# MCG-NJU/MotionRAG

Measured on AMD Instinct MI355X. Metric: denoise_step_frames_per_sec, higher is better.
Workload: dtype bf16

## Files before the change

### motionrag_amd/csrc/gemm_common.h

```cpp
#pragma once
#include <type_traits>
#include "common.h"
#include "../../include/mrag_hip.h"

namespace {

struct GemmP {
  const bf16_t* A; const bf16_t* W; const bf16_t* bias; bf16_t* C; const bf16_t* resid;
  const bf16_t* gate0; const bf16_t* gate1;
  long long M, N, K, lda, ldw, ldc, ldr, rows_per_batch, split, gate_stride;
  int tiles_m, tiles_n, group_m, staged, tuning;
  const bf16_t* qg; const bf16_t* qb; const bf16_t* kg; const bf16_t* kb; const float* rcos; const float* rsin;
  long long qk_D; int rope_text_len, qk_first; float qk_eps, q_premul;
  int cv_H, cv_W, cv_Hi, cv_Wi, cv_Ho, cv_Wo, cv_stride, cv_up, cv_ctiles, cv_T, cv_pad;
  long long cv_C, cv_HW;
  float acc_scale;
  float* sk_part; unsigned* sk_ticket;
  int sk_main, sk_rem, sk_units, sk_maxparts;
  const bf16_t* lna_g; const bf16_t* lna_b; float lna_eps; int lna;
  int tile_limit;
  int wb_tiles_m;
  long long w_bstride;
  int cv_lds;
  int cv_tf;
  long long cv_fs;
};

constexpr int SK_CUS = 256, SK_TICKET_BYTES = 1024;
constexpr int SK_FLAG_OFF = 8 * 128 * 144;
constexpr int SKM_ROWS = 32;

__device__ __forceinline__ float sum8_dpp(float x) {
  x += __int_as_float(__builtin_amdgcn_update_dpp(0, __float_as_int(x), 0xB1, 0xF, 0xF, true));
  x += __int_as_float(__builtin_amdgcn_update_dpp(0, __float_as_int(x), 0x4E, 0xF, 0xF, true));
  x += __int_as_float(__builtin_amdgcn_update_dpp(0, __float_as_int(x), 0x141, 0xF, 0xF, true));
  return x;
}

__device__ __forceinline__ u32x4 qk_row_math(u32x4 val, const bool has_gamma, const bool has_beta, const float (&gam)[8], const float (&bet)[8], const float eps,
                                             const bool has_rope, const bool vid, const f32x4 (&t4)[4], const bool premul_on, const float premul) {
  float v[8];
#pragma unroll
  for (int e = 0; e < 4; ++e) { v[2 * e] = __uint_as_float(val[e] << 16); v[2 * e + 1] = __uint_as_float(val[e] & 0xffff0000u); }
  if (has_gamma) {
    float sum = 0.f;
#pragma unroll
    for (int e = 0; e < 8; ++e) sum += v[e];
    sum = sum8_dpp(sum);
    const float mean = sum * (1.0f / 64.0f);
    float sq = 0.f;
#pragma unroll
    for (int e = 0; e < 8; ++e) { v[e] -= mean; sq += v[e] * v[e]; }
    sq = sum8_dpp(sq);
    const float rstd = rsqrtf(sq * (1.0f / 64.0f) + eps);
#pragma unroll
    for (int e = 0; e < 8; ++e) v[e] = v[e] * rstd * gam[e];
    if (has_beta) {
#pragma unroll
      for (int e = 0; e < 8; ++e) v[e] += bet[e];
    }
  }
  if (has_rope) {
    const float cc[8] = {t4[0][0], t4[0][1], t4[0][2], t4[0][3], t4[1][0], t4[1][1], t4[1][2], t4[1][3]};
    const float ss[8] = {t4[2][0], t4[2][1], t4[2][2], t4[2][3], t4[3][0], t4[3][1], t4[3][2], t4[3][3]};
#pragma unroll
    for (int i2 = 0; i2 < 4; ++i2) {
      const float a = v[2 * i2], b2 = v[2 * i2 + 1];
      const float oa = a * cc[2 * i2] - b2 * ss[2 * i2];
      const float ob = b2 * cc[2 * i2 + 1] + a * ss[2 * i2 + 1];
      v[2 * i2] = vid ? oa : a;
      v[2 * i2 + 1] = vid ? ob : b2;
    }
  }
  if (premul_on) {
#pragma unroll
    for (int e = 0; e < 8; ++e) v[e] *= premul;
  }
#pragma unroll
  for (int e = 0; e < 4; ++e) val[e] = pack_bf2(v[2 * e], v[2 * e + 1]);
  return val;
}

constexpr int EPI_GEGLU_TANH = 8;
template <int EPI>
constexpr bool is_geglu = (EPI == MRAG_EPI_GEGLU || EPI == EPI_GEGLU_TANH);

template <int EPI>
__device__ __forceinline__ float epi_act(float v) {
  if constexpr (EPI == MRAG_EPI_GELU_TANH) return gelu_tanh_f(v);
  else if constexpr (EPI == MRAG_EPI_GELU_ERF) return gelu_erf_f(v);
  else if constexpr (EPI == MRAG_EPI_SILU) return silu_f(v);
  else return v;
}


inline bool rows_16B_aligned(const void* C, long long ldc, const void* resid, long long ldr) {
  return ldc % 8 == 0 && ((uintptr_t)C & 15) == 0 && (!resid || (ldr % 8 == 0 && ((uintptr_t)resid & 15) == 0));
}

inline int group_m_of(int tuning) { return ((tuning >> 8) & 0xff) ? ((tuning >> 8) & 0xff) : 4; }

template <class P>
inline int launch_dyn_lds(void (*kernel)(P), dim3 grid, dim3 block, size_t lds_bytes, hipStream_t stream, const P& params) {
  const hipError_t e = hipFuncSetAttribute((const void*)kernel, hipFuncAttributeMaxDynamicSharedMemorySize, (int)lds_bytes);
  if (e != hipSuccess) return (int)e;
  MRAG_LAUNCH(kernel, grid, block, lds_bytes, stream, params);
  return (int)hipGetLastError();
}

inline bool wide_n_pays(long long N, int tuning = 0) {
  if (tuning & MRAG_GEMM_TUNE_NO_WIDE) return false;
  const long long w256 = (N + 255) / 256 * 256, w320 = (N + 319) / 320 * 320;
  return w320 * 100 < w256 * 90;
}

inline long long round_cost(long long M, long long N, int BN) {
  const long long tiles = ((M + 255) / 256) * ((N + BN - 1) / BN);
  return ((tiles + 255) / 256) * BN;
}
inline bool wide_rounds_pay(long long M, long long N, int tuning = 0, bool tail_rect = false) {
  if (tuning & MRAG_GEMM_TUNE_NO_WIDE) return false;
  long long c256 = round_cost(M, N, 256);
  if (tail_rect) c256 = (((M + 255) / 256) * ((N + 255) / 256) / 256) * 256 + 128;
  return round_cost(M, N, 320) * 100 < c256 * 85;
}
inline bool short_rows_pay(long long M, long long N, int tuning = 0) {
  if (tuning & MRAG_GEMM_TUNE_NO_WIDE) return false;
  const long long t192 = ((M + 191) / 192) * ((N + 255) / 256), t256 = ((M + 255) / 256) * ((N + 255) / 256);
  const long long c192 = ((t192 + 255) / 256) * 192 * 108, c256 = ((t256 + 255) / 256) * 256 * 100;
  return c192 * 100 < c256 * 90 && round_cost(M, N, 320) * 100 >= round_cost(M, N, 256) * 85;
}

inline bool narrow_n_pays(long long N) {
  const long long r = N % 256;
  return r != 0 && r <= 128;
}

struct SkPlan {
  bool use = false;
  int n_main = 0, rem = 0, units = 0, maxparts = 0;
  size_t bytes = 0;
};
inline SkPlan plan_streamk(long long M, long long N, long long K) {
  SkPlan pl;
  const long long tiles = ((M + 255) / 256) * ((N + 255) / 256);
  const int nk = (int)(K / 64);
  if (tiles < SK_CUS || tiles > (1 << 24) || nk < 16 || nk > 4096) return pl;
  const int rem = (int)(tiles % SK_CUS);
  if (rem == 0 || rem > 208) return pl;
  pl.rem = rem; pl.n_main = (int)(tiles - rem);
  pl.units = rem * 4 < SK_CUS ? rem * 4 : SK_CUS;
  const long long I = (long long)rem * nk;
  for (int t = 0, u = 0; t < rem; ++t) {
    while ((long long)(u + 1) * I / pl.units <= (long long)t * nk) ++u;
    int v = u;
    while ((long long)(v + 1) * I / pl.units < (long long)(t + 1) * nk) ++v;
    pl.maxparts = pl.maxparts > v - u + 1 ? pl.maxparts : v - u + 1;
  }
  pl.bytes = SK_TICKET_BYTES + (size_t)rem * pl.maxparts * 256 * 256 * sizeof(float);
  pl.use = true;
  return pl;
}

constexpr int W4_TAIL_MAX = 32;
inline bool tail_rect_wanted(long long tiles, int epi, int tuning) {
  const int rem = (int)(tiles % SK_CUS);
  return (tuning & MRAG_GEMM_TUNE_TAIL_RECT) && tiles >= 2 * SK_CUS && rem != 0 && rem <= W4_TAIL_MAX &&
         (epi == MRAG_EPI_NONE || epi == MRAG_EPI_GELU_TANH || epi == MRAG_EPI_RESID);
}

enum { TILE_256x256_W16, TILE_128x128, TILE_256x320, TILE_256x256 };

}

#define MRAG_GEMM_LAUNCHER extern "C" __attribute__((visibility("hidden"))) int
MRAG_GEMM_LAUNCHER launch_tiled(hipStream_t s, const GemmP& p, int epi, int tile, const SkPlan* sk);
MRAG_GEMM_LAUNCHER launch_w4(hipStream_t s, const GemmP& p, int epi);
MRAG_GEMM_LAUNCHER launch_k320(hipStream_t s, const GemmP& p, int epi);
MRAG_GEMM_LAUNCHER launch_skinny(hipStream_t s, const GemmP& p, int epi);
```

### motionrag_amd/csrc/gemm_w4.hip

```cpp
#include "gemm_common.h"

namespace {

template <int EPI>
__device__ __forceinline__ void epilogue_w4(const GemmP& p, char* smem, f32x4 (&acc)[8][8], const long long bm0, const long long bn0, const int wave, const int wrow0,
                                            const int wcol0, const int lane_in, const long long Mend) {
  constexpr bool HAS_R = (EPI == MRAG_EPI_GATE_RESID || EPI == MRAG_EPI_RESID), HAS_G = (EPI == MRAG_EPI_GATE_RESID), QK = (EPI == MRAG_EPI_QKNORM_ROPE);
  int lane_e = lane_in;
  asm volatile("" : "+v"(lane_e));
  const int lane = lane_e;
  const int frag_row = lane & 15, frag_q = lane >> 4;
  const long long n0 = bn0 + wcol0 + frag_q * 4;
  const long long m0 = bm0 + wrow0;
  long long g_b = 0, g_pos = 0;
  if constexpr (HAS_G || QK) {
    g_b = m0 / p.rows_per_batch;
    g_pos = m0 - g_b * p.rows_per_batch;
  }
  if (m0 >= Mend || bn0 + wcol0 >= p.N) return;
  const int mrows = (int)(Mend - m0 < 128 ? Mend - m0 : 128);
  bool fast = p.staged && bn0 + wcol0 + 128 <= p.N;
  if constexpr (HAS_G) fast = fast && g_pos + mrows - 1 < p.rows_per_batch && ((g_pos < p.split) == (g_pos + mrows - 1 < p.split));
  auto add_resid = [&](u32x2 out, const u32x2 r2) __attribute__((always_inline)) -> u32x2 {
    out[0] = pack_bf2(__uint_as_float(out[0] << 16) + __uint_as_float(r2[0] << 16), __uint_as_float(out[0] & 0xffff0000u) + __uint_as_float(r2[0] & 0xffff0000u));
    out[1] = pack_bf2(__uint_as_float(out[1] << 16) + __uint_as_float(r2[1] << 16), __uint_as_float(out[1] & 0xffff0000u) + __uint_as_float(r2[1] & 0xffff0000u));
    return out;
  };
  auto acc_math = [&](const int i, const int j, const u32x2 b2, const u32x2 g2) __attribute__((always_inline)) -> u32x2 {
    float v[4] = {acc[i][j][0], acc[i][j][1], acc[i][j][2], acc[i][j][3]};
    v[0] += __uint_as_float(b2[0] << 16); v[1] += __uint_as_float(b2[0] & 0xffff0000u);
    v[2] += __uint_as_float(b2[1] << 16); v[3] += __uint_as_float(b2[1] & 0xffff0000u);
    if constexpr (EPI == MRAG_EPI_GELU_TANH) {
      const f32x2 lo = gelu_tanh_f2(f32x2{v[0], v[1]}), hi = gelu_tanh_f2(f32x2{v[2], v[3]});
      v[0] = lo[0]; v[1] = lo[1]; v[2] = hi[0]; v[3] = hi[1];
    } else {
#pragma unroll
      for (int e = 0; e < 4; ++e) v[e] = epi_act<EPI>(v[e]);
    }
    if constexpr (HAS_G) {
      v[0] *= __uint_as_float(g2[0] << 16); v[1] *= __uint_as_float(g2[0] & 0xffff0000u);
      v[2] *= __uint_as_float(g2[1] << 16); v[3] *= __uint_as_float(g2[1] & 0xffff0000u);
    }
    if constexpr (EPI == MRAG_EPI_RESID) {
#pragma unroll
      for (int e = 0; e < 4; ++e) v[e] *= p.acc_scale;
    }
    return u32x2{pack_bf2(v[0], v[1]), pack_bf2(v[2], v[3])};
  };
  if (fast) {
    u32x2 bias[8], gate[8];
#pragma unroll
    for (int j = 0; j < 8; ++j) {
      bias[j] = p.bias ? *(const u32x2*)(p.bias + n0 + 16 * j) : u32x2{0u, 0u};
      if constexpr (HAS_G) gate[j] = *(const u32x2*)((g_pos < p.split ? p.gate0 : p.gate1) + g_b * p.gate_stride + n0 + 16 * j);
      else gate[j] = u32x2{0u, 0u};
    }
    const int r4 = lane >> 4, chunk = lane & 15;
    const bf16_t* rbase = HAS_R ? p.resid + m0 * p.ldr + n0 : nullptr;
    bf16_t* cbase = p.C + (m0 + r4) * p.ldc + (bn0 + wcol0 + chunk * 8);
    char* wput = smem + 131072 + wave * 8192 + frag_row * 256 + (frag_q & 1) * 8;
    const char* wget = smem + 131072 + wave * 8192 + r4 * 256;
    const int xput = frag_q >> 1;
    int qk_which = 2;
    bool has_rope = false;
    const bf16_t *gm = nullptr, *bt = nullptr;
    float gam[8], bet[8];
    f32x4 qk_tab[QK ? 3 : 1][4];
    unsigned qk_video = 0;
    auto qk_fetch = [&](const int st) __attribute__((always_inline)) {
      if constexpr (QK) {
        const int row = 4 * st + r4;
        long long pos = g_pos + (row < mrows ? row : mrows - 1);
        while (pos >= p.rows_per_batch) pos -= p.rows_per_batch;
        const int rp = (int)pos - p.rope_text_len;
        if (rp >= 0) qk_video |= 1u << st;
        const long long ro = (long long)(rp > 0 ? rp : 0) * 64 + (chunk & 7) * 8;
        f32x4(&dst)[4] = qk_tab[st % 3];
        dst[0] = *(const f32x4*)(p.rcos + ro); dst[1] = *(const f32x4*)(p.rcos + ro + 4);
        dst[2] = *(const f32x4*)(p.rsin + ro); dst[3] = *(const f32x4*)(p.rsin + ro + 4);
      }
    };
    if constexpr (QK) {
      qk_which = p.qk_first + (int)((bn0 + wcol0) / p.qk_D);
      has_rope = p.rcos != nullptr && qk_which < 2;
#pragma unroll
      for (int e = 0; e < 8; ++e) { gam[e] = 1.f; bet[e] = 0.f; }
      if (qk_which < 2) {
        gm = qk_which ? p.kg : p.qg;
        bt = qk_which ? p.kb : p.qb;
        const int d0 = (chunk & 7) * 8;
        if (gm) {
          const u32x4 graw = *(const u32x4*)(gm + d0);
#pragma unroll
          for (int e = 0; e < 4; ++e) { gam[2 * e] = __uint_as_float(graw[e] << 16); gam[2 * e + 1] = __uint_as_float(graw[e] & 0xffff0000u); }
          if (bt) {
            const u32x4 braw = *(const u32x4*)(bt + d0);
#pragma unroll
            for (int e = 0; e < 4; ++e) { bet[2 * e] = __uint_as_float(braw[e] << 16); bet[2 * e + 1] = __uint_as_float(braw[e] & 0xffff0000u); }
          }
        }
      }
      if (has_rope) { qk_fetch(0); qk_fetch(1); qk_fetch(2); }
    }
    constexpr int RD = 2;
    u32x2 rr[RD][8];
    auto fetch = [&](const int i, const int slot) __attribute__((always_inline)) {
      if constexpr (HAS_R) {
        const int row = 16 * i + frag_row;
        const bf16_t* rrow = rbase + (long long)(row < mrows ? row : mrows - 1) * p.ldr;
#pragma unroll
        for (int j = 0; j < 8; ++j) rr[slot][j] = *(const u32x2*)(rrow + 16 * j);
      }
    };
    auto put = [&](const int i) __attribute__((always_inline)) {
#pragma unroll
      for (int j = 0; j < 8; ++j) {
        u32x2 out = acc_math(i, j, bias[j], gate[j]);
        if constexpr (HAS_R) out = add_resid(out, rr[i % RD][j]);
        *(u32x2*)(wput + (i & 1) * 4096 + (((2 * j + xput) ^ frag_row) * 16)) = out;
      }
    };
    auto get_store = [&](const int i) __attribute__((always_inline)) {
      u32x4 val[4];
#pragma unroll
      for (int q = 0; q < 4; ++q) val[q] = *(const u32x4*)(wget + (i & 1) * 4096 + q * 1024 + ((chunk ^ (q * 4 + r4)) * 16));
#pragma unroll
      for (int q = 0; q < 4; ++q) {
        if constexpr (QK) {
          const int st = 4 * i + q;
          if (qk_which < 2) {
            val[q] = qk_row_math(val[q], gm != nullptr, bt != nullptr, gam, bet, p.qk_eps, has_rope, (qk_video >> st) & 1u, qk_tab[st % 3], qk_which == 0 && p.q_premul != 1.0f, p.q_premul);
            if (has_rope && st + 3 < 32) qk_fetch(st + 3);
          }
        }
        if (16 * i + 4 * q + r4 < mrows) *(u32x4*)(cbase + (long long)(16 * i + 4 * q) * p.ldc) = val[q];
      }
    };
#pragma unroll
    for (int i = 0; i < RD - 1; ++i) fetch(i, i);
#pragma unroll
    for (int i = 0; i < 8; ++i) {
      __builtin_amdgcn_sched_barrier(0);
      if (i + RD - 1 < 8) fetch(i + RD - 1, (i + RD - 1) % RD);
      put(i);
      if (i > 0) get_store(i - 1);
    }
    __builtin_amdgcn_sched_barrier(0);
    get_store(7);
    return;
  }
  if constexpr (QK) return;
  auto ncol = [&](const int j) __attribute__((always_inline)) { const long long n = n0 + 16 * j; return n < p.N ? n : p.N - 4; };
#pragma unroll
  for (int i = 0; i < 8; ++i) {
    __builtin_amdgcn_sched_barrier(0);
    const long long m = m0 + i * 16 + frag_row;
    const bool mok = m < Mend;
    const long long mc = mok ? m : Mend - 1;
    const bf16_t* gate = nullptr;
    if constexpr (HAS_G) {
      long long b = g_b, pos = g_pos + (mc - m0);
      while (pos >= p.rows_per_batch) { pos -= p.rows_per_batch; ++b; }
      gate = (pos < p.split ? p.gate0 : p.gate1) + b * p.gate_stride;
    }
#pragma unroll
    for (int j = 0; j < 8; ++j) {
      const long long n = ncol(j);
      const u32x2 b2 = p.bias ? *(const u32x2*)(p.bias + n) : u32x2{0u, 0u};
      u32x2 g2 = u32x2{0u, 0u};
      if constexpr (HAS_G) g2 = *(const u32x2*)(gate + n);
      u32x2 out = acc_math(i, j, b2, g2);
      if constexpr (HAS_R) out = add_resid(out, *(const u32x2*)(p.resid + mc * p.ldr + n));
      if (mok && n0 + 16 * j < p.N) *(u32x2*)(p.C + mc * p.ldc + n) = out;
    }
  }
  __builtin_amdgcn_s_waitcnt(0x0070);
}

template <int EPI>
__device__ __forceinline__ void epilogue_w4_geglu(const GemmP& p, char* smem, f32x4 (&acc)[8][8], const long long bm0, const long long bn0, const int wave, const int wrow0,
                                                  const int wcol0, const int lane_in) {
  int lane_e = lane_in;
  asm volatile("" : "+v"(lane_e));
  const int lane = lane_e;
  const int frag_row = lane & 15, frag_q = lane >> 4;
  const long long m0 = bm0 + wrow0;
  if (m0 >= p.M || bn0 + wcol0 >= p.N) return;
  const int mrows = (int)(p.M - m0 < 128 ? p.M - m0 : 128);
  const long long n0 = bn0 + wcol0 + frag_q * 4;
  u32x2 bv[4], bg[4];
#pragma unroll
  for (int jj = 0; jj < 4; ++jj) {
    bv[jj] = p.bias ? *(const u32x2*)(p.bias + n0 + 32 * jj) : u32x2{0u, 0u};
    bg[jj] = p.bias ? *(const u32x2*)(p.bias + n0 + 32 * jj + 16) : u32x2{0u, 0u};
  }
  const int r8 = lane >> 3, chunk = lane & 7;
  bf16_t* cbase = p.C + (m0 + r8) * p.ldc + ((bn0 + wcol0) >> 1) + chunk * 8;
  char* wput = smem + 131072 + wave * 8192 + frag_row * 128 + (frag_q & 1) * 8;
  const char* wget = smem + 131072 + wave * 8192 + r8 * 128 + ((chunk ^ r8) * 16);
  const int xput = frag_q >> 1, sw = frag_row & 7;
  auto put = [&](const int i) __attribute__((always_inline)) {
#pragma unroll
    for (int jj = 0; jj < 4; ++jj) {
      float v[4] = {acc[i][2 * jj][0], acc[i][2 * jj][1], acc[i][2 * jj][2], acc[i][2 * jj][3]};
      float g[4] = {acc[i][2 * jj + 1][0], acc[i][2 * jj + 1][1], acc[i][2 * jj + 1][2], acc[i][2 * jj + 1][3]};
      v[0] += __uint_as_float(bv[jj][0] << 16); v[1] += __uint_as_float(bv[jj][0] & 0xffff0000u);
      v[2] += __uint_as_float(bv[jj][1] << 16); v[3] += __uint_as_float(bv[jj][1] & 0xffff0000u);
      g[0] += __uint_as_float(bg[jj][0] << 16); g[1] += __uint_as_float(bg[jj][0] & 0xffff0000u);
      g[2] += __uint_as_float(bg[jj][1] << 16); g[3] += __uint_as_float(bg[jj][1] & 0xffff0000u);
      geglu4<EPI == EPI_GEGLU_TANH>(v, g);
      *(u32x2*)(wput + (i & 1) * 2048 + (((2 * jj + xput) ^ sw) * 16)) = u32x2{pack_bf2(v[0], v[1]), pack_bf2(v[2], v[3])};
    }
  };
  auto get_store = [&](const int i) __attribute__((always_inline)) {
    u32x4 val[2];
#pragma unroll
    for (int q = 0; q < 2; ++q) val[q] = *(const u32x4*)(wget + (i & 1) * 2048 + q * 1024);
#pragma unroll
    for (int q = 0; q < 2; ++q)
      if (16 * i + 8 * q + r8 < mrows) *(u32x4*)(cbase + (long long)(16 * i + 8 * q) * p.ldc) = val[q];
  };
#pragma unroll
  for (int i = 0; i < 8; ++i) {
    __builtin_amdgcn_sched_barrier(0);
    put(i);
    if (i > 0) get_store(i - 1);
  }
  __builtin_amdgcn_sched_barrier(0);
  get_store(7);
}

template <int N, class F>
__device__ __forceinline__ void static_for(F&& f) {
  if constexpr (N > 0) {
    static_for<N - 1>(f);
    f(std::integral_constant<int, N - 1>{});
  }
}

__device__ __forceinline__ void tile_coords(const GemmP& p, const int L, int& tile_m, int& tile_n) {
  const int gw = p.group_m * p.tiles_n;
  const int first_m = (L / gw) * p.group_m;
  const int gsz = min(p.tiles_m - first_m, p.group_m);
  tile_m = first_m + (L % gw) % gsz;
  tile_n = (L % gw) / gsz;
}

template <int EPI, bool WB = false>
__global__ __launch_bounds__(256) void gemm_w4_kernel(const GemmP p) {
  extern __shared__ __attribute__((aligned(16))) char smem[];
  constexpr unsigned STAGE = 65536, WOFF = 32768;
  const int lane = threadIdx.x & 63, wave = threadIdx.x >> 6, wm = wave >> 1, wn = wave & 1;
  const int wave_s = __builtin_amdgcn_readfirstlane(wave);
  const int tiles = p.tile_limit, nk = (int)(p.K / 64), G = (int)gridDim.x;
  auto tile_origin = [&](const int tm, long long& bm0, long long& m_end, long long& w_off) __attribute__((always_inline)) {
    if constexpr (WB) {
      const int b = tm / p.wb_tiles_m;
      bm0 = (long long)b * p.rows_per_batch + (long long)(tm - b * p.wb_tiles_m) * 256;
      m_end = (long long)(b + 1) * p.rows_per_batch;
      w_off = (long long)b * p.w_bstride;
    } else {
      bm0 = (long long)tm * 256; m_end = p.M; w_off = 0;
    }
  };
  const int slot = xcd_remap((int)blockIdx.x, G);
  unsigned voff[16];
  const bf16_t *baseA = p.A, *baseW = p.W;
  int d_r = 0, d_kt = 0;
  bool d_valid = false;
  auto cursor_set = [&](const int r) __attribute__((always_inline)) {
    const int L = r * G + slot;
    d_valid = L < tiles;
    if (!d_valid) return;
    int tm, tn;
    tile_coords(p, L, tm, tn);
    long long bm0, m_end, w_off;
    tile_origin(tm, bm0, m_end, w_off);
    const long long bn0 = (long long)tn * 256;
    int lane_c = lane;
    asm volatile("" : "+v"(lane_c));
    const int prow = lane_c >> 3, pchk = (lane_c & 7) ^ prow;
#pragma unroll
    for (int i = 0; i < 16; ++i) {
      const int q = wave_s + 4 * i;
      long long r8 = (i < 8) ? 8 * q + prow : 8 * (q - 32) + prow;
      const long long lim = (i < 8) ? m_end - bm0 : p.N - bn0;
      r8 = r8 < lim ? r8 : lim - 1;
      voff[i] = (unsigned)((r8 * ((i < 8) ? p.lda : p.ldw) + pchk * 8) * 2);
    }
    baseA = p.A + bm0 * p.lda;
    baseW = p.W + w_off + bn0 * p.ldw;
  };
  auto advance = [&]() __attribute__((always_inline)) {
    if (!d_valid) return;
    if (d_kt + 1 < nk) { ++d_kt; return; }
    cursor_set(d_r + 1);
    if (d_valid) { ++d_r; d_kt = 0; }
  };
  const unsigned smem_u = (unsigned)(size_t)smem;
  const unsigned fr = lane & 15, fq = lane >> 4, swz = lane & 7;
  const unsigned c0 = ((fq + 0) ^ swz) * 16, c1 = ((fq + 4) ^ swz) * 16;
  const unsigned rowA = smem_u + (wm * 128 + fr) * 128, rowW = smem_u + WOFF + (wn * 128 + fr) * 128;
  f32x4 acc[8][8];
  u32x4 a0[8], w0[8], a1[8], w1[8];
#define MRAG_W4_MF(I, J, W, A) asm volatile("v_mfma_f32_16x16x32_bf16 %0, %1, %2, %0" : "+a"(acc[I][J]) : "v"(W[J]), "v"(A[I]))
#define MRAG_W4_RD(D, ADDR, OFF) asm volatile("ds_read_b128 %0, %1 offset:%2" : "=v"(D) : "v"(ADDR), "n"(OFF) : "memory")
#define MRAG_W4_LGKM0(W, A)                                                                                          \
      asm volatile("s_waitcnt lgkmcnt(0)"                                                                             \
                   : "+v"(W[0]), "+v"(W[1]), "+v"(W[2]), "+v"(W[3]), "+v"(W[4]), "+v"(W[5]), "+v"(W[6]), "+v"(W[7]),   \
                     "+v"(A[0]), "+v"(A[1]), "+v"(A[2]), "+v"(A[3]), "+v"(A[4]), "+v"(A[5]), "+v"(A[6]), "+v"(A[7])    \
                   :: "memory")
  unsigned aw1, aa1, aw0, aa0, stage_u;
  auto dma = [&](auto I) __attribute__((always_inline)) {
    constexpr int i = decltype(I)::value;
    (void)&voff;
    const bf16_t* sb = (i < 8 ? baseA : baseW) + (long long)d_kt * 64;
    const unsigned lds = stage_u + (unsigned)(wave_s + 4 * i) * 1024u;
    asm volatile("s_mov_b32 m0, %2\n\ts_nop 0\n\tglobal_load_lds_dwordx4 %0, %1" :: "v"(voff[i]), "s"(sb), "s"(lds) : "memory", "m0");
  };
  auto kstep = [&](const unsigned g, const bool counted) __attribute__((always_inline)) {
    const unsigned so = (g & 1) ? STAGE : 0u, sn = STAGE - so;
    aw1 = rowW + so + c1; aa1 = rowA + so + c1;
    aw0 = rowW + sn + c0; aa0 = rowA + sn + c0;
    stage_u = smem_u + so;
    MRAG_W4_LGKM0(w0, a0);
    static_for<32>([&](auto S) __attribute__((always_inline)) {
      constexpr int sl = decltype(S)::value, i = (2 * sl) / 8, j = (2 * sl) % 8;
      (void)&acc; (void)&w0; (void)&a0; (void)&w1; (void)&a1; (void)&aw1; (void)&aa1;
      MRAG_W4_MF(i, j, w0, a0);
      if constexpr (sl < 8) MRAG_W4_RD(w1[sl], aw1, sl * 2048);
      else if constexpr (sl < 16) MRAG_W4_RD(a1[sl - 8], aa1, (sl - 8) * 2048);
      else if constexpr (sl == 22) { MRAG_W4_LGKM0(w1, a1); asm volatile("s_barrier" ::: "memory"); }
      else if constexpr (sl >= 23 && (sl & 1)) dma(std::integral_constant<int, (sl - 23) / 2>{});
      MRAG_W4_MF(i, j + 1, w0, a0);
    });
    if (counted) asm volatile("s_waitcnt vmcnt(5)" ::: "memory");
    asm volatile("s_barrier" ::: "memory");
    static_for<32>([&](auto S) __attribute__((always_inline)) {
      constexpr int sl = decltype(S)::value, i = (2 * sl) / 8, j = (2 * sl) % 8;
      (void)&acc; (void)&w0; (void)&a0; (void)&w1; (void)&a1; (void)&aw0; (void)&aa0;
      MRAG_W4_MF(i, j, w1, a1);
      if constexpr (sl < 8) MRAG_W4_RD(w0[sl], aw0, sl * 2048);
      else if constexpr (sl < 16) MRAG_W4_RD(a0[sl - 8], aa0, (sl - 8) * 2048);
      else if constexpr (sl >= 16 && sl < 27) dma(std::integral_constant<int, sl - 11>{});
      MRAG_W4_MF(i, j + 1, w1, a1);
    });
  };
  cursor_set(0);
  if (!d_valid) return;
  stage_u = smem_u;
  static_for<16>([&](auto I) __attribute__((always_inline)) { dma(I); });
  advance();
  stage_u = smem_u + STAGE;
  static_for<16>([&](auto I) __attribute__((always_inline)) { dma(I); });
  advance();
  asm volatile("s_waitcnt vmcnt(16)\n\ts_barrier" ::: "memory");
  aw0 = rowW + c0; aa0 = rowA + c0;
  static_for<8>([&](auto J) __attribute__((always_inline)) { constexpr int j = decltype(J)::value; (void)&w0; (void)&aw0; MRAG_W4_RD(w0[j], aw0, j * 2048); });
  static_for<8>([&](auto J) __attribute__((always_inline)) { constexpr int j = decltype(J)::value; (void)&a0; (void)&aa0; MRAG_W4_RD(a0[j], aa0, j * 2048); });
  unsigned g = 0;
  for (int r = 0;; ++r) {
    const int L = r * G + slot;
    if (L >= tiles) break;
#pragma unroll
    for (int i = 0; i < 8; ++i)
#pragma unroll
      for (int j = 0; j < 8; ++j) acc[i][j] = f32x4{0.f, 0.f, 0.f, 0.f};
    asm volatile("s_nop 4" ::: "memory");
    for (int t = 0; t < nk; ++t, ++g) {
      kstep(g, !(t == 0 && r > 0));
      advance();
    }
    asm volatile("s_waitcnt vmcnt(0)\n\ts_nop 15\n\ts_nop 15\n\ts_nop 7" ::: "memory");
    int tm, tn;
    tile_coords(p, L, tm, tn);
    long long e_bm0, e_mend, e_woff;
    tile_origin(tm, e_bm0, e_mend, e_woff);
    if constexpr (is_geglu<EPI>) epilogue_w4_geglu<EPI>(p, smem, acc, e_bm0, (long long)tn * 256, wave, wm * 128, wn * 128, lane);
    else epilogue_w4<EPI>(p, smem, acc, e_bm0, (long long)tn * 256, wave, wm * 128, wn * 128, lane, e_mend);
  }
#undef MRAG_W4_MF
#undef MRAG_W4_RD
#undef MRAG_W4_LGKM0
}

struct TailRect { bool use = false; int limit = 0; long long r0 = 0, c0 = 0; };
inline TailRect plan_tail_rect(const GemmP& p, int epi) {
  TailRect t;
  const long long tiles = (long long)p.tiles_m * p.tiles_n;
  if (p.wb_tiles_m || !tail_rect_wanted(tiles, epi, p.tuning)) return t;
  const int rem = (int)(tiles % SK_CUS);
  const int first_m = ((p.tiles_m - 1) / p.group_m) * p.group_m, gsz = p.tiles_m - first_m;
  const int ncols = (rem + gsz - 1) / gsz;
  if (ncols > p.tiles_n) return t;
  t.use = true;
  t.limit = (int)(tiles - (long long)gsz * ncols);
  t.r0 = (long long)first_m * 256; t.c0 = (long long)(p.tiles_n - ncols) * 256;
  return t;
}

}

extern "C" int launch_w4(hipStream_t s, const GemmP& p0, int epi) {
  if (256LL * (p0.lda > p0.ldw ? p0.lda : p0.ldw) * 2 >= (1LL << 32)) return MRAG_ENOTSUP;
  GemmP p = p0;
  const bool wb = p.w_bstride != 0;
  if (wb) {
    if (epi != MRAG_EPI_NONE || p.rows_per_batch <= 0 || p.M % p.rows_per_batch != 0) return MRAG_ENOTSUP;
    p.wb_tiles_m = (int)((p.rows_per_batch + 255) / 256);
    p.tiles_m = (int)(p.M / p.rows_per_batch) * p.wb_tiles_m;
  } else {
    p.wb_tiles_m = 0;
    p.tiles_m = (int)((p.M + 255) / 256);
  }
  p.tiles_n = (int)((p.N + 255) / 256);
  p.group_m = group_m_of(p.tuning);
  const long long tiles = (long long)p.tiles_m * p.tiles_n;
  p.staged = rows_16B_aligned(p.C, p.ldc, p.resid, p.ldr);
  if (p.tuning & MRAG_GEMM_TUNE_NO_STAGED) p.staged = 0;
  const TailRect tail = plan_tail_rect(p, epi);
  p.tile_limit = tail.use ? tail.limit : (int)tiles;
  const dim3 grid((unsigned)(p.tile_limit < SK_CUS ? p.tile_limit : SK_CUS)), block(256);
  const size_t lds = 131072 + 32768;
  int rc;
  switch (epi) {
    case MRAG_EPI_NONE:
      rc = wb ? launch_dyn_lds(gemm_w4_kernel<MRAG_EPI_NONE, true>, grid, block, lds, s, p) : launch_dyn_lds(gemm_w4_kernel<MRAG_EPI_NONE>, grid, block, lds, s, p);
      break;
    case MRAG_EPI_GELU_TANH: rc = launch_dyn_lds(gemm_w4_kernel<MRAG_EPI_GELU_TANH>, grid, block, lds, s, p); break;
    case MRAG_EPI_RESID: rc = launch_dyn_lds(gemm_w4_kernel<MRAG_EPI_RESID>, grid, block, lds, s, p); break;
    case MRAG_EPI_GATE_RESID: rc = launch_dyn_lds(gemm_w4_kernel<MRAG_EPI_GATE_RESID>, grid, block, lds, s, p); break;
    case MRAG_EPI_GEGLU:
    case EPI_GEGLU_TANH:
      if (!p.staged || p.N % 128 != 0) return MRAG_ENOTSUP;
      rc = epi == MRAG_EPI_GEGLU ? launch_dyn_lds(gemm_w4_kernel<MRAG_EPI_GEGLU>, grid, block, lds, s, p) : launch_dyn_lds(gemm_w4_kernel<EPI_GEGLU_TANH>, grid, block, lds, s, p);
      break;
    case MRAG_EPI_QKNORM_ROPE:
      if (!p.staged || p.N % 128 != 0 || p.qk_D % 128 != 0) return MRAG_ENOTSUP;
      rc = launch_dyn_lds(gemm_w4_kernel<MRAG_EPI_QKNORM_ROPE>, grid, block, lds, s, p);
      break;
    default: return MRAG_ENOTSUP;
  }
  if (rc != MRAG_OK) return rc;
  MRAG_COUNT(epi == MRAG_EPI_QKNORM_ROPE ? MRAG_K_GEMM_W4_QKNORM_ROPE : (epi == MRAG_EPI_GEGLU || epi == EPI_GEGLU_TANH) ? MRAG_K_GEMM_W4_GEGLU : wb ? MRAG_K_GEMM_W4_BATCHED_W : MRAG_K_GEMM_W4);
  if (tail.use) {
    GemmP t = p0;
    t.A = p0.A + tail.r0 * p0.lda; t.W = p0.W + tail.c0 * p0.ldw; t.C = p0.C + tail.r0 * p0.ldc + tail.c0;
    if (p0.bias) t.bias = p0.bias + tail.c0;
    if (p0.resid) t.resid = p0.resid + tail.r0 * p0.ldr + tail.c0;
    t.M = p0.M - tail.r0; t.N = p0.N - tail.c0;
    rc = launch_tiled(s, t, epi, TILE_128x128, nullptr);
    if (rc != MRAG_OK) return rc;
    MRAG_COUNT(MRAG_K_GEMM_W4_TAIL_RECT);
  }
  return MRAG_OK;
}
```

### motionrag_amd/csrc/norm.hip

```cpp
#include "common.h"
#include "../../include/mrag_hip.h"

constexpr int LN_STREAM_WGS = 2;

namespace {

__device__ __forceinline__ float wave_sum(float v) {
#pragma unroll
  for (int o = 32; o > 0; o >>= 1) v += __shfl_xor(v, o);
  return v;
}

__device__ __forceinline__ void unpack8(const u32x4 r, float* f) {
#pragma unroll
  for (int i = 0; i < 4; ++i) {
    f[2 * i] = __uint_as_float(r[i] << 16);
    f[2 * i + 1] = __uint_as_float(r[i] & 0xffff0000u);
  }
}
__device__ __forceinline__ u32x4 pack8(const float* f) {
  u32x4 r;
#pragma unroll
  for (int i = 0; i < 4; ++i) r[i] = pack_bf2(f[2 * i], f[2 * i + 1]);
  return r;
}

struct LnP {
  const bf16_t* x; bf16_t* y; const bf16_t* gamma; const bf16_t* beta;
  const bf16_t* shift0; const bf16_t* scale0; const bf16_t* shift1; const bf16_t* scale1;
  long long rows, D, ldx, ldy, rows_per_batch, split, mod_stride, y_rpb, y_bstride;
  float eps;
  int rms;
};

template <int MAXC>
__global__ __launch_bounds__(256) void layernorm_kernel(const LnP p) {
  const int lane = threadIdx.x & 63, wave = threadIdx.x >> 6;
  const long long row = (long long)blockIdx.x * 4 + wave;
  if (row >= p.rows) return;
  const bf16_t* x = p.x + row * p.ldx;
  float v[MAXC][8];
  float sum = 0.f;
#pragma unroll
  for (int c = 0; c < MAXC; ++c) {
    const long long idx = ((long long)c * 64 + lane) * 8;
    if (idx < p.D) {
      unpack8(__builtin_nontemporal_load((const u32x4*)(x + idx)), v[c]);
#pragma unroll
      for (int e = 0; e < 8; ++e) sum += v[c][e];
    } else {
#pragma unroll
      for (int e = 0; e < 8; ++e) v[c][e] = 0.f;
    }
  }
  const float mean = p.rms ? 0.f : wave_sum(sum) / (float)p.D;
  float sq = 0.f;
#pragma unroll
  for (int c = 0; c < MAXC; ++c) {
    const long long idx = ((long long)c * 64 + lane) * 8;
    if (idx < p.D) {
#pragma unroll
      for (int e = 0; e < 8; ++e) { const float d = __fsub_rn(v[c][e], mean); sq = __builtin_fmaf(d, d, sq); }
    }
  }
  const float rstd = rsqrtf(wave_sum(sq) / (float)p.D + p.eps);

  const bf16_t* shift = nullptr; const bf16_t* scale = nullptr;
  if (p.shift0) {
    const unsigned b = (unsigned)row / (unsigned)p.rows_per_batch, pos = (unsigned)row - b * (unsigned)p.rows_per_batch;
    shift = ((long long)pos < p.split ? p.shift0 : p.shift1) + (long long)b * p.mod_stride;
    scale = ((long long)pos < p.split ? p.scale0 : p.scale1) + (long long)b * p.mod_stride;
  }
  bf16_t* y = p.y_rpb > 0 ? p.y + (long long)((unsigned)row / (unsigned)p.y_rpb) * p.y_bstride + (long long)((unsigned)row % (unsigned)p.y_rpb) * p.ldy : p.y + row * p.ldy;
#pragma unroll
  for (int c = 0; c < MAXC; ++c) {
    const long long idx = ((long long)c * 64 + lane) * 8;
    if (idx >= p.D) continue;
    float o[8];
#pragma unroll
    for (int e = 0; e < 8; ++e) o[e] = __fmul_rn(__fsub_rn(v[c][e], mean), rstd);
    if (p.gamma) {
      float g[8]; unpack8(*(const u32x4*)(p.gamma + idx), g);
#pragma unroll
      for (int e = 0; e < 8; ++e) o[e] = __fmul_rn(o[e], g[e]);
    }
    if (p.beta) {
      float bb[8]; unpack8(*(const u32x4*)(p.beta + idx), bb);
#pragma unroll
      for (int e = 0; e < 8; ++e) o[e] = __fadd_rn(o[e], bb[e]);
    }
    if (shift) {
      float sc[8], sh[8];
      unpack8(*(const u32x4*)(scale + idx), sc);
      unpack8(*(const u32x4*)(shift + idx), sh);
#pragma unroll
      for (int e = 0; e < 8; ++e) o[e] = __builtin_fmaf(o[e], __fadd_rn(1.0f, sc[e]), sh[e]);
    }
    __builtin_nontemporal_store(pack8(o), (u32x4*)(y + idx));
  }
}

template <int MAXC>
__global__ __launch_bounds__(256, LN_STREAM_WGS) void layernorm_stream_kernel(const LnP p) {
  const int lane = threadIdx.x & 63;
  const long long nw = (long long)gridDim.x * 4, gw = (long long)blockIdx.x * 4 + (threadIdx.x >> 6);
  if (gw >= p.rows) return;
  u32x4 pg[MAXC], pb[MAXC], psc[MAXC], psh[MAXC];
  long long key_now = -1;
  u32x4 cur[MAXC], nxt[MAXC];
  auto load_row = [&](const long long row, u32x4 (&dst)[MAXC]) {
    const bf16_t* x = p.x + row * p.ldx + lane * 8;
#pragma unroll
    for (int c = 0; c < MAXC; ++c) dst[c] = __builtin_nontemporal_load((const u32x4*)(x + c * 512));
  };
  load_row(gw, nxt);
#pragma unroll
  for (int c = 0; c < MAXC; ++c) {
    const int idx = (c * 64 + lane) * 8;
    pg[c] = p.gamma ? *(const u32x4*)(p.gamma + idx) : u32x4{0u, 0u, 0u, 0u};
    pb[c] = p.beta ? *(const u32x4*)(p.beta + idx) : u32x4{0u, 0u, 0u, 0u};
    psc[c] = u32x4{0u, 0u, 0u, 0u}; psh[c] = u32x4{0u, 0u, 0u, 0u};
  }
  for (long long row = gw; row < p.rows; row += nw) {
#pragma unroll
    for (int c = 0; c < MAXC; ++c) cur[c] = nxt[c];
    if (row + nw < p.rows) load_row(row + nw, nxt);
    if (p.shift0) {
      const unsigned b = (unsigned)row / (unsigned)p.rows_per_batch, pos = (unsigned)row - b * (unsigned)p.rows_per_batch;
      const bool second = (long long)pos >= p.split;
      const long long key = 2LL * b + (second ? 1 : 0);
      if (key != key_now) {
        key_now = key;
        const bf16_t* shift = (second ? p.shift1 : p.shift0) + (long long)b * p.mod_stride;
        const bf16_t* scale = (second ? p.scale1 : p.scale0) + (long long)b * p.mod_stride;
#pragma unroll
        for (int c = 0; c < MAXC; ++c) {
          const int idx = (c * 64 + lane) * 8;
          psc[c] = *(const u32x4*)(scale + idx);
          psh[c] = *(const u32x4*)(shift + idx);
        }
      }
    }
    float sum = 0.f;
#pragma unroll
    for (int c = 0; c < MAXC; ++c) {
      float v[8]; unpack8(cur[c], v);
#pragma unroll
      for (int e = 0; e < 8; ++e) sum += v[e];
    }
    const float mean = p.rms ? 0.f : wave_sum(sum) / (float)p.D;
    float sq = 0.f;
#pragma unroll
    for (int c = 0; c < MAXC; ++c) {
      float v[8]; unpack8(cur[c], v);
#pragma unroll
      for (int e = 0; e < 8; ++e) { const float d = __fsub_rn(v[e], mean); sq = __builtin_fmaf(d, d, sq); }
    }
    const float rstd = rsqrtf(wave_sum(sq) / (float)p.D + p.eps);
    bf16_t* y = p.y + row * p.ldy + lane * 8;
#pragma unroll
    for (int c = 0; c < MAXC; ++c) {
      float v[8], o[8]; unpack8(cur[c], v);
#pragma unroll
      for (int e = 0; e < 8; ++e) o[e] = __fmul_rn(__fsub_rn(v[e], mean), rstd);
      if (p.gamma) {
        float g[8]; unpack8(pg[c], g);
#pragma unroll
        for (int e = 0; e < 8; ++e) o[e] = __fmul_rn(o[e], g[e]);
      }
      if (p.beta) {
        float bb[8]; unpack8(pb[c], bb);
#pragma unroll
        for (int e = 0; e < 8; ++e) o[e] = __fadd_rn(o[e], bb[e]);
      }
      if (p.shift0) {
        float sc[8], sh[8]; unpack8(psc[c], sc); unpack8(psh[c], sh);
#pragma unroll
        for (int e = 0; e < 8; ++e) o[e] = __builtin_fmaf(o[e], __fadd_rn(1.0f, sc[e]), sh[e]);
      }
      __builtin_nontemporal_store(pack8(o), (u32x4*)(y + c * 512));
    }
  }
}

template <int LPR, int CH>
__global__ __launch_bounds__(256) void layernorm_rows_kernel(const LnP p) {
  constexpr int RPW = 64 / LPR;
  const int lane = threadIdx.x & 63, wave = threadIdx.x >> 6, sub = lane % LPR, rs = lane / LPR;
  const long long row0 = ((long long)blockIdx.x * 4 + wave) * RPW + rs;
  const long long row = row0 < p.rows ? row0 : p.rows - 1;
  const bf16_t* x = p.x + row * p.ldx;
  float v[CH][8];
  float sum = 0.f;
#pragma unroll
  for (int c = 0; c < CH; ++c) {
    unpack8(__builtin_nontemporal_load((const u32x4*)(x + (sub + LPR * c) * 8)), v[c]);
#pragma unroll
    for (int e = 0; e < 8; ++e) sum += v[c][e];
  }
#pragma unroll
  for (int o = LPR / 2; o > 0; o >>= 1) sum += __shfl_xor(sum, o);
  const float mean = sum / (float)p.D;
  float sq = 0.f;
#pragma unroll
  for (int c = 0; c < CH; ++c)
#pragma unroll
    for (int e = 0; e < 8; ++e) { const float d = v[c][e] - mean; sq += d * d; }
#pragma unroll
  for (int o = LPR / 2; o > 0; o >>= 1) sq += __shfl_xor(sq, o);
  const float rstd = rsqrtf(sq / (float)p.D + p.eps);
  bf16_t* y = p.y_rpb > 0 ? p.y + (long long)((unsigned)row / (unsigned)p.y_rpb) * p.y_bstride + (long long)((unsigned)row % (unsigned)p.y_rpb) * p.ldy : p.y + row * p.ldy;
#pragma unroll
  for (int c = 0; c < CH; ++c) {
    const int idx = (sub + LPR * c) * 8;
    float o[8];
#pragma unroll
    for (int e = 0; e < 8; ++e) o[e] = (v[c][e] - mean) * rstd;
    if (p.gamma) {
      float g[8]; unpack8(*(const u32x4*)(p.gamma + idx), g);
#pragma unroll
      for (int e = 0; e < 8; ++e) o[e] *= g[e];
    }
    if (p.beta) {
      float bb[8]; unpack8(*(const u32x4*)(p.beta + idx), bb);
#pragma unroll
      for (int e = 0; e < 8; ++e) o[e] += bb[e];
    }
    if (row0 < p.rows) __builtin_nontemporal_store(pack8(o), (u32x4*)(y + idx));
  }
}

struct QkP {
  bf16_t* qkv; const bf16_t* qg; const bf16_t* qb; const bf16_t* kg; const bf16_t* kb;
  const float* cos; const float* sin;
  int B, S, H, text_len; float eps, q_premul;
};

__global__ __launch_bounds__(256) void qknorm_rope_kernel(const QkP p) {
  const int lane = threadIdx.x & 63, wave = threadIdx.x >> 6;
  const int hgroups = (p.H + 7) / 8;
  const long long units = (long long)p.B * p.S * 2 * hgroups;
  const int sub = lane >> 3, d0 = (lane & 7) * 8;
  for (long long u = (long long)blockIdx.x * 4 + wave; u < units; u += (long long)gridDim.x * 4) {
    const int hg = (int)(u % hgroups);
    const int which = (int)((u / hgroups) & 1);
    const long long tok = u / (2 * hgroups);
    const int s = (int)(tok % p.S);
    const int head = hg * 8 + sub;
    if (head >= p.H) continue;
    bf16_t* ptr = p.qkv + tok * (3LL * p.H * 64) + (long long)which * p.H * 64 + head * 64 + d0;
    float v[8];
    unpack8(*(const u32x4*)ptr, v);
    const bf16_t* g = which ? p.kg : p.qg;
    const bf16_t* bt = which ? p.kb : p.qb;
    if (g) {
      float sum = 0.f;
#pragma unroll
      for (int e = 0; e < 8; ++e) sum += v[e];
      sum += __shfl_xor(sum, 1); sum += __shfl_xor(sum, 2); sum += __shfl_xor(sum, 4);
      const float mean = sum * (1.0f / 64.0f);
      float sq = 0.f;
#pragma unroll
      for (int e = 0; e < 8; ++e) { v[e] -= mean; sq += v[e] * v[e]; }
      sq += __shfl_xor(sq, 1); sq += __shfl_xor(sq, 2); sq += __shfl_xor(sq, 4);
      const float rstd = rsqrtf(sq * (1.0f / 64.0f) + p.eps);
      float gg[8], bb[8];
      unpack8(*(const u32x4*)(g + d0), gg);
#pragma unroll
      for (int e = 0; e < 8; ++e) v[e] = v[e] * rstd * gg[e];
      if (bt) {
        unpack8(*(const u32x4*)(bt + d0), bb);
#pragma unroll
        for (int e = 0; e < 8; ++e) v[e] += bb[e];
      }
    }
    if (p.cos && s >= p.text_len) {
      const long long ro = (long long)(s - p.text_len) * 64 + d0;
      const f32x4 c0 = *(const f32x4*)(p.cos + ro), c1 = *(const f32x4*)(p.cos + ro + 4);
      const f32x4 s0 = *(const f32x4*)(p.sin + ro), s1 = *(const f32x4*)(p.sin + ro + 4);
      const float cc[8] = {c0[0], c0[1], c0[2], c0[3], c1[0], c1[1], c1[2], c1[3]};
      const float ss[8] = {s0[0], s0[1], s0[2], s0[3], s1[0], s1[1], s1[2], s1[3]};
      float o[8];
#pragma unroll
      for (int i = 0; i < 4; ++i) {
        o[2 * i] = v[2 * i] * cc[2 * i] - v[2 * i + 1] * ss[2 * i];
        o[2 * i + 1] = v[2 * i + 1] * cc[2 * i + 1] + v[2 * i] * ss[2 * i + 1];
      }
#pragma unroll
      for (int e = 0; e < 8; ++e) v[e] = o[e];
    }
    if (!which && p.q_premul != 1.0f) {
#pragma unroll
      for (int e = 0; e < 8; ++e) v[e] *= p.q_premul;
    }
    *(u32x4*)ptr = pack8(v);
  }
}

}

extern "C" int mrag_layernorm_bf16(void* stream, const mrag_ln_args* a) {
  if (!a || !a->x || !a->y || a->rows <= 0 || a->D <= 0) return MRAG_EINVAL;
  if (a->D % 8 != 0 || a->ldx % 8 != 0 || a->ldy % 8 != 0) return MRAG_EINVAL;
  if (((uintptr_t)a->x | (uintptr_t)a->y) & 15) return MRAG_EINVAL;
  if (a->D > 8192 || a->rows >= (1LL << 31) || a->rows_per_batch >= (1LL << 31) || a->y_rows_per_batch >= (1LL << 31)) return MRAG_ENOTSUP;
  if (a->shift0 && (!a->scale0 || !a->shift1 || !a->scale1 || a->rows_per_batch <= 0 || a->mod_stride % 8 != 0))
    return MRAG_EINVAL;
  LnP p{};
  p.x = (const bf16_t*)a->x; p.y = (bf16_t*)a->y; p.gamma = (const bf16_t*)a->gamma; p.beta = (const bf16_t*)a->beta;
  p.shift0 = (const bf16_t*)a->shift0; p.scale0 = (const bf16_t*)a->scale0;
  p.shift1 = (const bf16_t*)a->shift1; p.scale1 = (const bf16_t*)a->scale1;
  p.rows = a->rows; p.D = a->D; p.ldx = a->ldx; p.ldy = a->ldy;
  p.rows_per_batch = a->rows_per_batch; p.split = a->split; p.mod_stride = a->mod_stride; p.eps = a->eps; p.rms = a->rms;
  p.y_rpb = a->y_rows_per_batch; p.y_bstride = a->y_batch_stride;
  if (p.y_rpb < 0 || (p.y_rpb > 0 && p.y_bstride % 8 != 0)) return MRAG_EINVAL;
  const dim3 grid((unsigned)((a->rows + 3) / 4)), block(256);
  hipStream_t s = (hipStream_t)stream;
  if (!a->shift0 && !a->rms && (a->D == 320 || a->D == 640 || a->D == 1280 || a->D == 1024) && a->rows >= 1024) {
    if (a->D == 320) MRAG_LAUNCH((layernorm_rows_kernel<8, 5>), dim3((unsigned)((a->rows + 31) / 32)), block, 0, s, p);
    else if (a->D == 640) MRAG_LAUNCH((layernorm_rows_kernel<16, 5>), dim3((unsigned)((a->rows + 15) / 16)), block, 0, s, p);
    else if (a->D == 1024) MRAG_LAUNCH((layernorm_rows_kernel<16, 8>), dim3((unsigned)((a->rows + 15) / 16)), block, 0, s, p);
    else MRAG_LAUNCH((layernorm_rows_kernel<32, 5>), dim3((unsigned)((a->rows + 7) / 8)), block, 0, s, p);
    MRAG_LAUNCH_CHECK();
    MRAG_COUNT(MRAG_K_LAYERNORM_ROWS);
    return MRAG_OK;
  }
  if (a->D == 3072 && a->rows >= 8192 && p.y_rpb == 0) {
    MRAG_LAUNCH(layernorm_stream_kernel<6>, dim3(256 * LN_STREAM_WGS), block, 0, s, p);
    MRAG_LAUNCH_CHECK();
    MRAG_COUNT(MRAG_K_LAYERNORM_STREAM);
    return MRAG_OK;
  }
  if (a->D <= 1024) MRAG_LAUNCH(layernorm_kernel<2>, grid, block, 0, s, p);
  else if (a->D <= 2048) MRAG_LAUNCH(layernorm_kernel<4>, grid, block, 0, s, p);
  else if (a->D <= 3072) MRAG_LAUNCH(layernorm_kernel<6>, grid, block, 0, s, p);
  else if (a->D <= 4096) MRAG_LAUNCH(layernorm_kernel<8>, grid, block, 0, s, p);
  else MRAG_LAUNCH(layernorm_kernel<16>, grid, block, 0, s, p);
  MRAG_LAUNCH_CHECK();
  MRAG_COUNT(MRAG_K_LAYERNORM);
  return MRAG_OK;
}

extern "C" int mrag_qknorm_rope_bf16(void* stream, const mrag_qknorm_rope_args* a) {
  if (!a || !a->qkv || a->B <= 0 || a->S <= 0 || a->H <= 0) return MRAG_EINVAL;
  if ((uintptr_t)a->qkv & 15) return MRAG_EINVAL;
  if ((a->cos == nullptr) != (a->sin == nullptr)) return MRAG_EINVAL;
  if (a->cos && (((uintptr_t)a->cos | (uintptr_t)a->sin) & 15)) return MRAG_EINVAL;
  if (a->text_len < 0 || a->text_len > a->S) return MRAG_EINVAL;
  QkP p{};
  p.qkv = (bf16_t*)a->qkv; p.qg = (const bf16_t*)a->q_gamma; p.qb = (const bf16_t*)a->q_beta;
  p.kg = (const bf16_t*)a->k_gamma; p.kb = (const bf16_t*)a->k_beta;
  p.cos = a->cos; p.sin = a->sin; p.B = a->B; p.S = a->S; p.H = a->H; p.text_len = a->text_len;
  p.eps = a->eps; p.q_premul = a->q_premul;
  const long long units = (long long)a->B * a->S * 2 * ((a->H + 7) / 8);
  long long blocks = (units + 3) / 4;
  if (blocks > 256 * 32) blocks = 256 * 32;
  MRAG_LAUNCH(qknorm_rope_kernel, dim3((unsigned)blocks), dim3(256), 0, (hipStream_t)stream, p);
  MRAG_LAUNCH_CHECK();
  MRAG_COUNT(MRAG_K_QKNORM_ROPE);
  return MRAG_OK;
}
```

Baseline: 88.58.

## Move residual add after LDS transpose with deep row-wise prefetch in w4 epilogue

The w4 GEMM fast-path epilogue now adds the residual after the LDS transpose, on full 16-byte row chunks, instead of on 8-byte fragments before it. Residual rows are prefetched eight store-steps ahead in a rolling register buffer. The rope and non-rope store paths become compile-time specialised. Accumulators are read explicitly from AGPRs, and fp contraction is disabled in the qk norm and rope math so results stay consistent between the fused GEMM path and the standalone norm kernel. This trades more live registers for fewer, wider, better-overlapped residual loads.

```diff
diff --git a/motionrag_amd/csrc/gemm_common.h b/motionrag_amd/csrc/gemm_common.h
--- a/motionrag_amd/csrc/gemm_common.h
+++ b/motionrag_amd/csrc/gemm_common.h
@@ -39,6 +39,7 @@
 
 __device__ __forceinline__ u32x4 qk_row_math(u32x4 val, const bool has_gamma, const bool has_beta, const float (&gam)[8], const float (&bet)[8], const float eps,
                                              const bool has_rope, const bool vid, const f32x4 (&t4)[4], const bool premul_on, const float premul) {
+#pragma clang fp contract(off)
   float v[8];
 #pragma unroll
   for (int e = 0; e < 4; ++e) { v[2 * e] = __uint_as_float(val[e] << 16); v[2 * e + 1] = __uint_as_float(val[e] & 0xffff0000u); }
@@ -52,7 +53,7 @@
 #pragma unroll
     for (int e = 0; e < 8; ++e) { v[e] -= mean; sq += v[e] * v[e]; }
     sq = sum8_dpp(sq);
-    const float rstd = rsqrtf(sq * (1.0f / 64.0f) + eps);
+    const float rstd = rsqrtf(__builtin_fmaf(sq, 1.0f / 64.0f, eps));
 #pragma unroll
     for (int e = 0; e < 8; ++e) v[e] = v[e] * rstd * gam[e];
     if (has_beta) {
diff --git a/motionrag_amd/csrc/gemm_w4.hip b/motionrag_amd/csrc/gemm_w4.hip
--- a/motionrag_amd/csrc/gemm_w4.hip
+++ b/motionrag_amd/csrc/gemm_w4.hip
@@ -21,13 +21,13 @@
   const int mrows = (int)(Mend - m0 < 128 ? Mend - m0 : 128);
   bool fast = p.staged && bn0 + wcol0 + 128 <= p.N;
   if constexpr (HAS_G) fast = fast && g_pos + mrows - 1 < p.rows_per_batch && ((g_pos < p.split) == (g_pos + mrows - 1 < p.split));
-  auto add_resid = [&](u32x2 out, const u32x2 r2) __attribute__((always_inline)) -> u32x2 {
-    out[0] = pack_bf2(__uint_as_float(out[0] << 16) + __uint_as_float(r2[0] << 16), __uint_as_float(out[0] & 0xffff0000u) + __uint_as_float(r2[0] & 0xffff0000u));
-    out[1] = pack_bf2(__uint_as_float(out[1] << 16) + __uint_as_float(r2[1] << 16), __uint_as_float(out[1] & 0xffff0000u) + __uint_as_float(r2[1] & 0xffff0000u));
-    return out;
+  auto add_bf2 = [](const unsigned o, const unsigned r) __attribute__((always_inline)) -> unsigned {
+    return pack_bf2(__uint_as_float(o << 16) + __uint_as_float(r << 16), __uint_as_float(o & 0xffff0000u) + __uint_as_float(r & 0xffff0000u));
   };
   auto acc_math = [&](const int i, const int j, const u32x2 b2, const u32x2 g2) __attribute__((always_inline)) -> u32x2 {
-    float v[4] = {acc[i][j][0], acc[i][j][1], acc[i][j][2], acc[i][j][3]};
+    float v[4];
+#pragma unroll
+    for (int e = 0; e < 4; ++e) asm volatile("v_accvgpr_read_b32 %0, %1" : "=v"(v[e]) : "a"(acc[i][j][e]));
     v[0] += __uint_as_float(b2[0] << 16); v[1] += __uint_as_float(b2[0] & 0xffff0000u);
     v[2] += __uint_as_float(b2[1] << 16); v[3] += __uint_as_float(b2[1] & 0xffff0000u);
     if constexpr (EPI == MRAG_EPI_GELU_TANH) {
@@ -56,16 +56,33 @@
       else gate[j] = u32x2{0u, 0u};
     }
     const int r4 = lane >> 4, chunk = lane & 15;
-    const bf16_t* rbase = HAS_R ? p.resid + m0 * p.ldr + n0 : nullptr;
     bf16_t* cbase = p.C + (m0 + r4) * p.ldc + (bn0 + wcol0 + chunk * 8);
     char* wput = smem + 131072 + wave * 8192 + frag_row * 256 + (frag_q & 1) * 8;
     const char* wget = smem + 131072 + wave * 8192 + r4 * 256;
     const int xput = frag_q >> 1;
+    constexpr int RR = 8;
+    const int tail_st = (mrows - 1) >> 2;
+    const bf16_t *rfull = nullptr, *rtail = nullptr;
+    u32x4 rres[HAS_R ? RR : 1];
+    auto rfetch = [&](const int st) __attribute__((always_inline)) {
+      if constexpr (HAS_R) {
+        rres[st % RR] = *(const u32x4*)(st < tail_st ? rfull : rtail);
+        rfull += 4 * p.ldr;
+      }
+    };
+    if constexpr (HAS_R) {
+      const int trow = 4 * tail_st + r4;
+      rfull = p.resid + (m0 + r4) * p.ldr + (bn0 + wcol0 + chunk * 8);
+      rtail = p.resid + (m0 + (trow < mrows ? trow : mrows - 1)) * p.ldr + (bn0 + wcol0 + chunk * 8);
+#pragma unroll
+      for (int st = 0; st < RR; ++st) rfetch(st);
+    }
+    constexpr int QR = 3;
     int qk_which = 2;
     bool has_rope = false;
     const bf16_t *gm = nullptr, *bt = nullptr;
     float gam[8], bet[8];
-    f32x4 qk_tab[QK ? 3 : 1][4];
+    f32x4 qk_tab[QK ? QR : 1][4];
     unsigned qk_video = 0;
     auto qk_fetch = [&](const int st) __attribute__((always_inline)) {
       if constexpr (QK) {
@@ -75,7 +92,7 @@
         const int rp = (int)pos - p.rope_text_len;
         if (rp >= 0) qk_video |= 1u << st;
         const long long ro = (long long)(rp > 0 ? rp : 0) * 64 + (chunk & 7) * 8;
-        f32x4(&dst)[4] = qk_tab[st % 3];
+        f32x4(&dst)[4] = qk_tab[st % QR];
         dst[0] = *(const f32x4*)(p.rcos + ro); dst[1] = *(const f32x4*)(p.rcos + ro + 4);
         dst[2] = *(const f32x4*)(p.rsin + ro); dst[3] = *(const f32x4*)(p.rsin + ro + 4);
       }
@@ -100,53 +117,54 @@
           }
         }
       }
-      if (has_rope) { qk_fetch(0); qk_fetch(1); qk_fetch(2); }
-    }
-    constexpr int RD = 2;
-    u32x2 rr[RD][8];
-    auto fetch = [&](const int i, const int slot) __attribute__((always_inline)) {
-      if constexpr (HAS_R) {
-        const int row = 16 * i + frag_row;
-        const bf16_t* rrow = rbase + (long long)(row < mrows ? row : mrows - 1) * p.ldr;
-#pragma unroll
-        for (int j = 0; j < 8; ++j) rr[slot][j] = *(const u32x2*)(rrow + 16 * j);
-      }
+      if (has_rope) {
+#pragma unroll
+        for (int st = 0; st < QR; ++st) qk_fetch(st);
+      }
+    }
+    auto put = [&](const int i) __attribute__((always_inline)) {
+#pragma unroll
+      for (int j = 0; j < 8; ++j) *(u32x2*)(wput + (i & 1) * 4096 + (((2 * j + xput) ^ frag_row) * 16)) = acc_math(i, j, bias[j], gate[j]);
     };
-    auto put = [&](const int i) __attribute__((always_inline)) {
-#pragma unroll
-      for (int j = 0; j < 8; ++j) {
-        u32x2 out = acc_math(i, j, bias[j], gate[j]);
-        if constexpr (HAS_R) out = add_resid(out, rr[i % RD][j]);
-        *(u32x2*)(wput + (i & 1) * 4096 + (((2 * j + xput) ^ frag_row) * 16)) = out;
-      }
-    };
-    auto get_store = [&](const int i) __attribute__((always_inline)) {
+    auto get_store = [&](const int i, auto ROPE) __attribute__((always_inline)) {
+      constexpr bool rope = decltype(ROPE)::value;
       u32x4 val[4];
 #pragma unroll
       for (int q = 0; q < 4; ++q) val[q] = *(const u32x4*)(wget + (i & 1) * 4096 + q * 1024 + ((chunk ^ (q * 4 + r4)) * 16));
 #pragma unroll
       for (int q = 0; q < 4; ++q) {
+        const int st = 4 * i + q;
         if constexpr (QK) {
-          const int st = 4 * i + q;
-          if (qk_which < 2) {
-            val[q] = qk_row_math(val[q], gm != nullptr, bt != nullptr, gam, bet, p.qk_eps, has_rope, (qk_video >> st) & 1u, qk_tab[st % 3], qk_which == 0 && p.q_premul != 1.0f, p.q_premul);
-            if (has_rope && st + 3 < 32) qk_fetch(st + 3);
+          if (rope || qk_which < 2) {
+            val[q] = qk_row_math(val[q], gm != nullptr, bt != nullptr, gam, bet, p.qk_eps, rope, (qk_video >> st) & 1u, qk_tab[st % QR], qk_which == 0 && p.q_premul != 1.0f, p.q_premul);
+            if (rope && st + QR < 32) qk_fetch(st + QR);
           }
         }
-        if (16 * i + 4 * q + r4 < mrows) *(u32x4*)(cbase + (long long)(16 * i + 4 * q) * p.ldc) = val[q];
+        if constexpr (HAS_R) {
+#pragma unroll
+          for (int e = 0; e < 4; ++e) val[q][e] = add_bf2(val[q][e], rres[st % RR][e]);
+        }
+        if constexpr (QK || HAS_R) asm volatile("" :: "v"(val[q]));
+        if (4 * st + r4 < mrows) *(u32x4*)(cbase + (long long)(4 * st) * p.ldc) = val[q];
+        if (st + RR < 32) rfetch(st + RR);
       }
     };
-#pragma unroll
-    for (int i = 0; i < RD - 1; ++i) fetch(i, i);
-#pragma unroll
-    for (int i = 0; i < 8; ++i) {
+    auto stores = [&](auto ROPE) __attribute__((always_inline)) {
+#pragma unroll
+      for (int i = 0; i < 8; ++i) {
+        __builtin_amdgcn_sched_barrier(0);
+        put(i);
+        if (i > 0) get_store(i - 1, ROPE);
+      }
       __builtin_amdgcn_sched_barrier(0);
-      if (i + RD - 1 < 8) fetch(i + RD - 1, (i + RD - 1) % RD);
-      put(i);
-      if (i > 0) get_store(i - 1);
-    }
-    __builtin_amdgcn_sched_barrier(0);
-    get_store(7);
+      get_store(7, ROPE);
+    };
+    if constexpr (QK) {
+      if (has_rope) stores(std::true_type{});
+      else stores(std::false_type{});
+    } else {
+      stores(std::false_type{});
+    }
     return;
   }
   if constexpr (QK) return;
@@ -170,7 +188,10 @@
       u32x2 g2 = u32x2{0u, 0u};
       if constexpr (HAS_G) g2 = *(const u32x2*)(gate + n);
       u32x2 out = acc_math(i, j, b2, g2);
-      if constexpr (HAS_R) out = add_resid(out, *(const u32x2*)(p.resid + mc * p.ldr + n));
+      if constexpr (HAS_R) {
+        const u32x2 r2 = *(const u32x2*)(p.resid + mc * p.ldr + n);
+        out = u32x2{add_bf2(out[0], r2[0]), add_bf2(out[1], r2[1])};
+      }
       if (mok && n0 + 16 * j < p.N) *(u32x2*)(p.C + mc * p.ldc + n) = out;
     }
   }
diff --git a/motionrag_amd/csrc/norm.hip b/motionrag_amd/csrc/norm.hip
--- a/motionrag_amd/csrc/norm.hip
+++ b/motionrag_amd/csrc/norm.hip
@@ -260,10 +260,13 @@
       sum += __shfl_xor(sum, 1); sum += __shfl_xor(sum, 2); sum += __shfl_xor(sum, 4);
       const float mean = sum * (1.0f / 64.0f);
       float sq = 0.f;
-#pragma unroll
-      for (int e = 0; e < 8; ++e) { v[e] -= mean; sq += v[e] * v[e]; }
+      {
+#pragma clang fp contract(off)
+#pragma unroll
+        for (int e = 0; e < 8; ++e) { v[e] -= mean; sq += v[e] * v[e]; }
+      }
       sq += __shfl_xor(sq, 1); sq += __shfl_xor(sq, 2); sq += __shfl_xor(sq, 4);
-      const float rstd = rsqrtf(sq * (1.0f / 64.0f) + p.eps);
+      const float rstd = rsqrtf(__builtin_fmaf(sq, 1.0f / 64.0f, p.eps));
       float gg[8], bb[8];
       unpack8(*(const u32x4*)(g + d0), gg);
 #pragma unroll
@@ -281,10 +284,13 @@
       const float cc[8] = {c0[0], c0[1], c0[2], c0[3], c1[0], c1[1], c1[2], c1[3]};
       const float ss[8] = {s0[0], s0[1], s0[2], s0[3], s1[0], s1[1], s1[2], s1[3]};
       float o[8];
-#pragma unroll
-      for (int i = 0; i < 4; ++i) {
-        o[2 * i] = v[2 * i] * cc[2 * i] - v[2 * i + 1] * ss[2 * i];
-        o[2 * i + 1] = v[2 * i + 1] * cc[2 * i + 1] + v[2 * i] * ss[2 * i + 1];
+      {
+#pragma clang fp contract(off)
+#pragma unroll
+        for (int i = 0; i < 4; ++i) {
+          o[2 * i] = v[2 * i] * cc[2 * i] - v[2 * i + 1] * ss[2 * i];
+          o[2 * i + 1] = v[2 * i + 1] * cc[2 * i + 1] + v[2 * i] * ss[2 * i + 1];
+        }
       }
 #pragma unroll
       for (int e = 0; e < 8; ++e) v[e] = o[e];
```

Result: faster. 90.60, median of 6 (+2.3%).
